# sadPororo/AD-YOLO

Hardware: AMD Instinct MI355X
Metric: train-step audio-sec/s (4ch, se-resnet34+adyolo) (higher is better)
Workload: dtype f32; 1 GPU; se-resnet34 + adyolo loss, synthetic 4ch 24kHz 60s clips, bs=64 per GPU, 12 classes, features+fwd+loss+bwd+allreduce+Adam; global_batch=64, parallelism=dp1

## Files before the change

ad-yolo_amd/_lib.py:

```python
import ctypes
import os

_HERE = os.path.dirname(os.path.abspath(__file__))
LIB_PATH = os.environ.get("ADYOLO_LIB") or os.path.join(_HERE, "libadyolo_hip.so")

P = ctypes.c_void_p
I = ctypes.c_int
L = ctypes.c_long
F = ctypes.c_float
U64 = ctypes.c_uint64

SIGNATURES = {
    "adyolo_abi_version": (I, []),
    "adyolo_last_error": (ctypes.c_char_p, []),
    "adyolo_feat_stft_mel": (I, [P] * 8 + [I, I] + [P] * 4 + [I, I, I, P]),
    "adyolo_feat_finish": (I, [P] * 4 + [I, I, I, P]),
    "adyolo_feat_gcc_phat": (I, [P] * 6 + [I, I, I, I, P]),
    "adyolo_nchw_to_nhwc8": (I, [P, P, I, I, I, I, P]),
    "adyolo_pack_w3x3": (I, [P, P, P, I, I, I, P]),
    "adyolo_conv3x3_tiles": (I, [I] * 3),
    "adyolo_conv3x3_fwd": (I, [P] * 13 + [I] * 7 + [P]),
    "adyolo_wino_pack_w": (I, [P, P, P, I, I, I, P]),
    "adyolo_wino_pack_many": (I, [P, I, I, I, P]),
    "adyolo_wino_tiles": (I, [I] * 3),
    "adyolo_wino_fwd": (I, [P] * 13 + [I] * 7 + [P]),
    "adyolo_wino4_pack_w": (I, [P, P, P, I, I, I, P]),
    "adyolo_wino4_pack_many": (I, [P, I, I, I, P]),
    "adyolo_wino4_tiles": (I, [I] * 3),
    "adyolo_wino4_fwd": (I, [P] * 13 + [I] * 7 + [P]),
    "adyolo_wino4_fwd_form": (I, [I] * 3),
    "adyolo_wino4_last_form": (I, []),
    "adyolo_set_switches": (I, [I]),
    "adyolo_wino4_wgrad_slabs": (I, [I] * 5),
    "adyolo_wino4_wgrad": (I, [P] * 7 + [I] * 6 + [P]),
    "adyolo_wino_wgrad_slabs": (I, [I] * 5),
    "adyolo_wino_wgrad": (I, [P] * 7 + [I] * 6 + [P]),
    "adyolo_conv3x3_wgrad_slabs": (I, [I] * 5),
    "adyolo_conv3x3_wgrad": (I, [P] * 6 + [I] * 6 + [P]),
    "adyolo_wgrad_plan": (I, [I] * 6 + [P]),
    "adyolo_conv_fwd_plan": (I, [I] * 9 + [P]),
    "adyolo_gemm": (I, [P] * 5 + [I] * 10 + [P]),
    "adyolo_gemm_plan": (I, [I] * 8 + [P, P, P]),
    "adyolo_gemm_batched": (I, [P] * 3 + [I] * 10 + [L] * 6 + [F, I, P]),
    "adyolo_colsum": (I, [P, P, P, I, I, I, I, P]),
    "adyolo_bn_stats": (I, [P] * 7 + [I, I, I, F, F, P]),
    "adyolo_bn_stats_tiles": (I, [P] * 11 + [I, I, I, I, F, F, P]),
    "adyolo_bn_eval_stats": (I, [P] * 4 + [I, F, P]),
    "adyolo_bn_scale_shift": (I, [P] * 6 + [I, P]),
    "adyolo_affine_nhwc": (I, [P] * 4 + [L, I, P]),
    "adyolo_bn_bwd_reduce": (I, [P] * 7 + [L, I, P]),
    "adyolo_bn_bwd_tiles": (I, [P, P, P, P, I, I, P]),
    "adyolo_bn_bwd_apply": (I, [P] * 12 + [L, I, I, F, P]),
    "adyolo_bn_persample": (I, [P, P, P, I, I, I, P]),
    "adyolo_bn_finish": (I, [P] * 10 + [I, I, I, F, F, P]),
    "adyolo_se_fc_fwd": (I, [P] * 10 + [I, I, I, I, P]),
    "adyolo_relu_mask_words": (L, [I, I, I]),
    "adyolo_se_tail_fwd": (I, [P] * 9 + [I, I, I, P]),
    "adyolo_se_tail_fwd_pool_ok": (I, [I, I, I]),
    "adyolo_se_tail_fwd_pool": (I, [P] * 9 + [I, I, I, I, P]),
    "adyolo_se_tail_bwd_reduce": (I, [P] * 9 + [I, I, I, P]),
    "adyolo_se_tail_bwd_tiles": (I, [P, P, P, I, I, I, P]),
    "adyolo_se_fc_bwd_words": (L, [I, I]),
    "adyolo_se_fc_bwd": (I, [P] * 16 + [I, I, I, I, P]),
    "adyolo_se_tail_bwd_apply": (I, [P] * 13 + [I, I, I, F, P]),
    "adyolo_se_tail_bwd_reduce_pooled": (I, [P] * 8 + [I, I, I, I, P]),
    "adyolo_se_tail_bwd_apply_pooled": (I, [P] * 13 + [I, I, I, I, F, P]),
    "adyolo_avgpool2_fwd": (I, [P, P, I, I, I, I, P]),
    "adyolo_avgpool2_bwd": (I, [P, P, I, I, I, I, P]),
    "adyolo_add": (I, [P, P, P, L, P]),
    "adyolo_mul": (I, [P, P, P, L, P]),
    "adyolo_scale_dev": (I, [P, P, P, L, P]),
# ... 145 lines not shown
```

ad-yolo_amd/csrc/conv.hip:

```cpp
#include <stdlib.h>
#include "common.hpp"

namespace adyolo {

template <int KC, int BN, int TW>
struct ConvCfg {
    static constexpr int TH = 256 / TW;
    static constexpr int HW_ = TW + 2;
    static constexpr int HH_ = TH + 2;
    static constexpr int NPIX = HW_ * HH_;
    static constexpr int AS = KC + 4;
    static constexpr int NT = BN / 32;
    static constexpr int Q = KC / 4;
    static constexpr int A_FLOATS = NPIX * AS;
    static constexpr int W_FLOATS = BN * AS;
    static constexpr int WPT = (BN * Q + 255) / 256;
};

template <int KC, int BN, int TW>
__global__ __launch_bounds__(256, 2) void conv3x3_fwd_kernel(
    const float *__restrict__ x, const float *__restrict__ wpk, const float *__restrict__ bias,
    const float *__restrict__ addend, const float *__restrict__ addend_mask, const float *__restrict__ in_scale,
    const float *__restrict__ in_shift, float *__restrict__ y, float *__restrict__ stats,
    const float *__restrict__ stat_aux, const float *__restrict__ stat_mean, const float *__restrict__ stat_invstd,
// ... 372 lines not shown
                    float sq = v * v;
                    asm volatile("" : "+v"(sq));
                    ssq += sq;
                }
            }
            float *yrow = y + (((size_t)n * H + gy) * W + tx0) * 32;
#pragma unroll
            for (int k = 0; k < 4; ++k) {
                const int px = k * 8 + (lane >> 3), c4 = lane & 7;
                const f32x4 v4 = *reinterpret_cast<const f32x4 *>(&ot[px * 36 + c4 * 4]);
                if (tx0 + px < W) __builtin_nontemporal_store(v4, reinterpret_cast<f32x4 *>(yrow + (size_t)px * 32 + c4 * 4));
            }
        }
    }
    if (stats) {
        const float a0 = ssum + __shfl_xor(ssum, 32, 64), a1 = ssq + __shfl_xor(ssq, 32, 64);
        if (lh == 0) {
            red[(wave * 32 + li) * 2 + 0] = a0;
            red[(wave * 32 + li) * 2 + 1] = a1;
        }
        __syncthreads();
        if (tid < 64) {
            const int c = tid >> 1, which = tid & 1;
            const float v = red[(0 * 32 + c) * 2 + which] + red[(1 * 32 + c) * 2 + which] + red[(2 * 32 + c) * 2 + which] +
                            red[(3 * 32 + c) * 2 + which];
            stats[which * ((size_t)gridDim.x * 32) + (size_t)blockIdx.x * 32 + c] = v;
        }
    }
}

constexpr int SW_U = 8;
constexpr int SW_T = 64;
constexpr int SW_XS = (SW_T + 4) * 8;
__global__ __launch_bounds__(256, 2) void stem_wgrad_kernel(const float *__restrict__ x, const float *__restrict__ dy,
                                                            float *__restrict__ slabs, int H, int W, int rows_total) {
    __shared__ __attribute__((aligned(16))) float lds[4 * SW_T * 32 + 7 * SW_XS];
    static_assert(4 * SW_T * 32 + 7 * SW_XS >= 4 * 32 * 72, "the reduction buffer must fit");
    float *dyL = lds, *xL = lds + 4 * SW_T * 32;
    const int tid = threadIdx.x, lane = tid & 63, wave = tid >> 6;
    const int li = lane & 31, lh = lane >> 5;
    int ky[3], boff[3];
#pragma unroll
    for (int t = 0; t < 3; ++t) {
        const int n = t * 32 + li, tap = n < 72 ? n >> 3 : 8;
        ky[t] = tap / 3 - 1;
        boff[t] = (lh + 1 + (tap % 3 - 1)) * 8 + (n & 7);
    }
    f32x16 acc[3];
#pragma unroll
    for (int t = 0; t < 3; ++t)
#pragma unroll
        for (int r = 0; r < 16; ++r) acc[t][r] = 0.f;
    for (int i = tid; i < SW_XS; i += 256) xL[6 * SW_XS + i] = 0.f;

    const int per = (rows_total + gridDim.x - 1) / gridDim.x;
    const int r0 = blockIdx.x * per, r1 = min(rows_total, r0 + per);
    const int ncol = (W + SW_T - 1) / SW_T;
    const int nchunk = r0 < r1 ? ((r1 - r0 + 3) / 4) * ncol : 0;
    f32x4 pd[8], px_[4];
    auto request = [&](int chunk) {
        const int cr = r0 + (chunk / ncol) * 4, c0 = (chunk % ncol) * SW_T;
        const __amdgpu_buffer_rsrc_t drs = __builtin_amdgcn_make_buffer_rsrc(const_cast<float *>(dy) + (size_t)cr * W * 32, 0,
                                                                              0x7fffffff, 0x00020000);
        const __amdgpu_buffer_rsrc_t xrs = __builtin_amdgcn_make_buffer_rsrc(const_cast<float *>(x) + ((ptrdiff_t)cr - 1) * W * 8, 0,
                                                                              0x7fffffff, 0x00020000);
#pragma unroll
        for (int i = 0; i < 8; ++i) {
            const int f = tid + 256 * i;
            const int j = f >> 9, col = c0 + ((f & 511) >> 3);
            const bool ok = cr + j < r1 && col < W;
            pd[i] = __builtin_bit_cast(f32x4, __builtin_amdgcn_raw_buffer_load_b128(
                                                  drs, ok ? ((j * W + col) * 32 + (f & 7) * 4) * 4 : (int)0x80000000, 0, 0));
        }
#pragma unroll
        for (int i = 0; i < 4; ++i) {
            const int f = tid + 256 * i;
            const int j = f / 132, rem = f - j * 132;
            const int row = cr - 1 + j, col = c0 - 1 + (rem >> 1);
            const bool ok = f < 6 * 132 && row >= 0 && row < rows_total && col >= 0 && col < W;
            px_[i] = __builtin_bit_cast(f32x4, __builtin_amdgcn_raw_buffer_load_b128(
                                                   xrs, ok ? ((j * W + col) * 8 + (rem & 1) * 4) * 4 : (int)0x80000000, 0, 0));
        }
    };
    auto deposit = [&]() {
#pragma unroll
        for (int i = 0; i < 8; ++i) *reinterpret_cast<f32x4 *>(&dyL[(tid + 256 * i) * 4]) = pd[i];
#pragma unroll
        for (int i = 0; i < 4; ++i) {
            const int f = tid + 256 * i;
            const int j = f / 132;
            if (f < 6 * 132) *reinterpret_cast<f32x4 *>(&xL[j * SW_XS + (f - j * 132) * 4]) = px_[i];
        }
    };
    if (nchunk > 0) request(0);
    for (int chunk = 0; chunk < nchunk; ++chunk) {
        deposit();
        __syncthreads();
        if (chunk + 1 < nchunk) request(chunk + 1);
        const int row = r0 + (chunk / ncol) * 4 + wave;
        if (row < r1) {
            const int y = row % H;
            const float *ap = dyL + (wave * SW_T + lh) * 32 + li;
            const float *bp[3];
#pragma unroll
            for (int t = 0; t < 3; ++t) {
                const int yy = y + ky[t];
                bp[t] = xL + ((yy >= 0 && yy < H) ? wave + 1 + ky[t] : 6) * SW_XS + boff[t];
            }
            constexpr int NG = SW_T / (2 * SW_U);
            float a[2][SW_U], b[2][3][SW_U];
            auto reads = [&](int g) {
#pragma unroll
                for (int u = 0; u < SW_U; ++u) {
                    a[g & 1][u] = ap[(g * SW_U + u) * 64];
#pragma unroll
                    for (int t = 0; t < 3; ++t) b[g & 1][t][u] = bp[t][(g * SW_U + u) * 16];
                }
            };
            reads(0);
#pragma unroll
            for (int g = 0; g < NG; ++g) {
                __builtin_amdgcn_sched_barrier(0);
                if (g + 1 < NG) reads(g + 1);
                __builtin_amdgcn_sched_barrier(0);
#pragma unroll
                for (int u = 0; u < SW_U; ++u)
#pragma unroll
                    for (int t = 0; t < 3; ++t) acc[t] = mfma32(a[g & 1][u], b[g & 1][t][u], acc[t]);
            }
        }
        __syncthreads();
    }
    float *red = lds;
#pragma unroll
    for (int t = 0; t < 3; ++t)
#pragma unroll
        for (int r = 0; r < 16; ++r) {
            const int n = t * 32 + li;
            if (n < 72) red[(wave * 32 + mfma_row(r, lane)) * 72 + n] = acc[t][r];
        }
    __syncthreads();
    for (int i = tid; i < 32 * 72; i += 256)
        slabs[(size_t)blockIdx.x * (32 * 72) + i] = ((red[i] + red[32 * 72 + i]) + red[2 * 32 * 72 + i]) + red[3 * 32 * 72 + i];
}

__global__ __launch_bounds__(256) void conv3x3_wgrad_reduce_kernel(const float *__restrict__ slabs,
                                                                   float *__restrict__ dw, int nslab, int Cout,
                                                                   int CinP, int Cin_real) {
    __shared__ double red[256];
    const int total = Cout * 9 * CinP;
    const double sum = block_colsum32(slabs, nslab, (size_t)total, blockIdx.x * 32, total, red);
    const int idx = blockIdx.x * 32 + (threadIdx.x & 31);
    if ((threadIdx.x >> 5) != 0 || idx >= total) return;
    const int ci = idx % CinP;
    const int tap = (idx / CinP) % 9;
    const int co = idx / (CinP * 9);
    if (ci < Cin_real) dw[((size_t)co * Cin_real + ci) * 9 + tap] = (float)sum;
}

__global__ void pack_w3x3_kernel(const float *__restrict__ w, float *__restrict__ wf,
                                 float *__restrict__ wd, int Cout, int Cin_real, int Cin) {
    const int idx = blockIdx.x * blockDim.x + threadIdx.x;
    if (idx >= Cout * 9 * Cin) return;
    const int ci = idx % Cin;
    const int tap = (idx / Cin) % 9;
    const int co = idx / (Cin * 9);
    const float v = ci < Cin_real ? w[((size_t)co * Cin_real + ci) * 9 + tap] : 0.f;
    wf[idx] = v;
    if (wd) wd[((size_t)ci * 9 + (8 - tap)) * Cout + co] = v;
}

template <int KC, int BN, int TW>
static int launch_fwd(const float *x, const float *wpk, const float *bias, const float *addend,
                      const float *addend_mask, const float *in_scale, const float *in_shift, float *y, float *stats,
                      const float *stat_aux, const float *stat_mean, const float *stat_invstd, const float *stat_mask,
                      int N, int H, int W, int Cin, int Cout, int relu, int mask_bits, hipStream_t st, int tilesW, int tilesH) {
    dim3 grid((unsigned)(N * tilesH * tilesW), (unsigned)(Cout / BN));
    hipLaunchKernelGGL((conv3x3_fwd_kernel<KC, BN, TW>), grid, dim3(256), 0, st, x, wpk, bias, addend, addend_mask,
                       in_scale, in_shift, y, stats, stat_aux, stat_mean, stat_invstd, stat_mask, H, W, Cin, Cout, tilesW,
                       tilesH, relu, mask_bits);
    return check_launch("conv3x3_fwd");
}

static int wgrad_splits(int N, int H, int W, int Cin, int Cout, int *TWo) {
    const int TW = W >= 32 ? 32 : 16, TH = 256 / TW;
    const int ntiles = N * cdiv(H, TH) * cdiv(W, TW);
    const int blocks = (Cout / 32) * cdiv(Cin, 32);
    int nsplit = 1024 / blocks;
    if (nsplit < 1) nsplit = 1;
// ... 56 lines not shown
    hipStream_t st = as_stream(stream);
    const ConvFwdVariant v = conv3x3_fwd_variant(H, W, Cin, Cout, !addend && !in_scale && !stat_aux && !stat_mask);
#define ADYOLO_FWD(KC_, BN_, TW_) \
    launch_fwd<KC_, BN_, TW_>(x, wpk, bias, addend, addend_mask, in_scale, in_shift, y, stats, stat_aux, stat_mean, \
                              stat_invstd, stat_mask, N, H, W, Cin, Cout, relu, mask_bits, st, v.tilesW, v.tilesH)
    if (v.stem) {
        hipLaunchKernelGGL(stem_fwd_kernel, dim3((unsigned)(N * v.tilesH * v.tilesW)), dim3(256), 0, st, x, wpk, bias, y, stats, H,
                           W, v.tilesW, v.tilesH, relu);
        return check_launch("stem_fwd");
    }
    const bool wide = v.TW == 32;
    if (v.KC == 8) return wide ? ADYOLO_FWD(8, 32, 32) : ADYOLO_FWD(8, 32, 16);
    if (v.BN == 64) return wide ? ADYOLO_FWD(32, 64, 32) : ADYOLO_FWD(32, 64, 16);
    return wide ? ADYOLO_FWD(32, 32, 32) : ADYOLO_FWD(32, 32, 16);
#undef ADYOLO_FWD
}

extern "C" int adyolo_conv3x3_wgrad_slabs(int N, int H, int W, int Cin, int Cout) {
    if (N <= 0 || H <= 0 || W <= 0 || Cin <= 0 || Cout <= 0 || Cout % 32) return ADYOLO_EINVAL;
    return wgrad_splits(N, H, W, Cin, Cout, nullptr);
}

extern "C" int adyolo_conv3x3_wgrad(const float *x, const float *dy, const float *in_scale, const float *in_shift,
                                    float *slabs, float *dw, int N, int H, int W, int Cin, int Cin_real, int Cout,
                                    void *stream) {
    ADYOLO_REQUIRE(x && dy && slabs && dw && N > 0 && H > 0 && W > 0, ADYOLO_EINVAL, "conv3x3_wgrad: bad arguments");
    ADYOLO_REQUIRE((Cin == 8 || Cin % 32 == 0) && Cout % 32 == 0 && Cin_real <= Cin, ADYOLO_ENOSUP,
                   "conv3x3_wgrad: unsupported channels Cin=%d Cout=%d", Cin, Cout);
    hipStream_t st = as_stream(stream);
    int TW;
    const int nsplit = wgrad_splits(N, H, W, Cin, Cout, &TW);
    if (Cin == 8 && Cout == 32 && !in_scale && (long)N * H < (1L << 31)) {
        const int nblk = nsplit < 512 ? nsplit : 512;
        hipLaunchKernelGGL(stem_wgrad_kernel, dim3(nblk), dim3(256), 0, st, x, dy, slabs, H, W, N * H);
        int rcs = check_launch("stem_wgrad");
        if (rcs) return rcs;
        hipLaunchKernelGGL(conv3x3_wgrad_reduce_kernel, dim3(cdiv(32 * 72, 32)), dim3(256), 0, st, slabs, dw, nblk, 32, 8,
                           Cin_real);
        return check_launch("stem_wgrad_reduce");
    }
    const int TH = 256 / TW;
    const int tilesW = cdiv(W, TW), tilesH = cdiv(H, TH);
    const int ntiles = N * tilesW * tilesH;
    const int cinBlocks = cdiv(Cin, 32);
    dim3 grid((unsigned)nsplit, (unsigned)((Cout / 32) * cinBlocks));
    if (TW == 32)
        hipLaunchKernelGGL((conv3x3_wgrad_kernel<32>), grid, dim3(256), 0, st, x, dy, in_scale, in_shift, slabs, H, W,
                           Cin, Cout, tilesW, tilesH, ntiles, nsplit, cinBlocks);
    else
        hipLaunchKernelGGL((conv3x3_wgrad_kernel<16>), grid, dim3(256), 0, st, x, dy, in_scale, in_shift, slabs, H, W,
                           Cin, Cout, tilesW, tilesH, ntiles, nsplit, cinBlocks);
    int rc = check_launch("conv3x3_wgrad");
    if (rc) return rc;
    const int CinP = cinBlocks * 32;
    const int total = Cout * 9 * CinP;
    hipLaunchKernelGGL(conv3x3_wgrad_reduce_kernel, dim3(cdiv(total, 32)), dim3(256), 0, st, slabs, dw, nsplit,
                       Cout, CinP, Cin_real);
    return check_launch("conv3x3_wgrad_reduce");
}

extern "C" int adyolo_wgrad_plan(int form, int N, int H, int W, int Cin, int Cout, int *out8) {
    ADYOLO_REQUIRE(out8 && form >= 0 && form <= 3 && N > 0 && H > 0 && W > 0 && Cin > 0 && Cout > 0, ADYOLO_EINVAL,
                   "wgrad_plan: bad arguments");
    for (int i = 0; i < 8; ++i) out8[i] = 0;
    if (form <= 1) {
        if (Cout % 32 || (Cin != 8 && Cin % 32)) return 0;
        if (form == 1 && !(Cin == 8 && Cout == 32 && (long)N * H < (1L << 31))) return 0;
        int TW;
        const int nsplit = wgrad_splits(N, H, W, Cin, Cout, &TW);
        out8[0] = nsplit;
        out8[2] = 1;
        out8[4] = 1;
        if (form == 0) {
            out8[1] = N * cdiv(H, 256 / TW) * cdiv(W, TW);
            out8[3] = 256 / TW;
            out8[5] = TW;
        } else {
            const int nblk = nsplit < 512 ? nsplit : 512;
            out8[1] = N * H;
            out8[3] = cdiv(N * H, nblk);
            out8[5] = SW_T;
            out8[6] = nblk;
        }
        out8[7] = 1;
        return 0;
    }
    if (form == 2) {
        if (adyolo_wino_wgrad_slabs(N, H, W, Cin, Cout) <= 0 ||
            (size_t)H * W * (Cin > Cout ? Cin : Cout) * 4 >= ((size_t)1 << 31))
            return 0;
        wino_wgrad_plan(N, H, W, Cin, Cout, out8);
// ... 73 lines not shown
```

ad-yolo_amd/functional.py:

```python
import os
from typing import NamedTuple

import torch

from . import ops

FUSE_BNBWD = os.environ.get("ADYOLO_FUSE_BNBWD", "1") != "0"
FUSE_POOL = os.environ.get("ADYOLO_FUSE_POOL", "1") != "0"
FUSE_POOL_BWD = os.environ.get("ADYOLO_FUSE_POOL_BWD", "1") != "0"


class BlockLink:

    def __init__(self):
        self.cc = self.mean2 = self.invstd2 = self.tiles = self.ebits = None
        self.affine = self.stem_bn = None
        self.prepooled = None


class BlockArgs(NamedTuple):
    bn1: object
    bn2: object
    bnd: object = None
    link_in: object = None
# ... 157 lines not shown
        if training:
            a, st = ops.conv3x3(x8, wpk, w.shape[0], bias=b, relu=True, want_stats=True)
            _, mean, invstd, scale, shift = _BNState(bn).stats_tiles(st, a, affine=(gamma, beta))
        else:
            a = ops.conv3x3(x8, wpk, w.shape[0], bias=b, relu=True)
            mean, invstd, scale, shift = _BNState(bn).eval_affine(gamma, beta)
        ctx.holder = None
        if holder is not None:
            holder.affine = (scale, shift)
            if training and FUSE_BNBWD:
                holder.stem_bn = (a.detach(), mean, invstd)
                ctx.holder = holder
            out = a
        else:
            out = ops.affine(a, scale, shift)
        ctx.training = training
        ctx.cin_real = w.shape[1]
        ctx.ptrs = (w.data_ptr(), gamma.data_ptr(), beta.data_ptr())
        ctx.wshape = tuple(w.shape)
        ctx.saved_names = ["x8", "a", "gamma", "mean", "invstd"]
        ctx.save_for_backward(x8, a, gamma, mean, invstd)
        return out

    @staticmethod
    def backward(ctx, dout):
        if not ctx.training:
            raise NotImplementedError("backward through eval-mode BatchNorm is not part of the hot path")
        x8, a, gamma, mean, invstd = ctx.saved_tensors
        pw, pg, pb = ctx.ptrs
        vg, vb, vw = SINK.view(pg), SINK.view(pb), SINK.view(pw, ctx.wshape)
        tiles = None
        if ctx.holder is not None and ctx.holder.tiles is not None:
            tiles, ctx.holder.tiles = ctx.holder.tiles, None
        da, dgamma, dbeta, db = ops.bn_bwd(_c(dout), a, gamma, mean, invstd, relu_mask=True, tile_stats=tiles,
                                           out_dgamma=vg, out_dbeta=vb, want_dx_colsum=True)
        dw = ops.conv3x3_wgrad(x8, da, ctx.cin_real, out=vw)
        if vw is not None:
            SINK.done(pw, pg, pb)
            return None, None, db, None, None, None, None, None
        return None, dw, db, dgamma, dbeta, None, None, None


class SEBlockFn(torch.autograd.Function):

    @staticmethod
    def forward(ctx, x, training, pool, args, w1, g1, b1, w2, g2, b2, fw1, fb1, fw2, fb2, wd=None, gd=None, bd=None):
        link_in, link_out, p_aff = args.link_in, args.link_out, args.in_affine
        prepooled = pool and link_in is not None and link_in.prepooled is not None
        if prepooled and tuple(x.shape[1:3]) != link_in.prepooled:
            raise ValueError("SEBlockFn: link_in.prepooled says the block below wrote a %d x %d map, but the input is %d x %d"
                             % (link_in.prepooled + tuple(x.shape[1:3])))
        if p_aff is not None and (pool or wd is not None):
            raise NotImplementedError("p_affine is only supported for identity-shortcut blocks without pooling")
        p = ops.avgpool2(x) if (pool and not prepooled) else x
        n, h, w_, cin = p.shape
        c = w1.shape[0]
        if args.packs is not None:
            wpk1, wpk1d, wpk2, wpk2d = args.packs
        else:
            wpk1, wpk1d = ops.pack_w3x3(w1, cin)
            wpk2, wpk2d = ops.pack_w3x3(w2, c)
        if training:
            a, st1 = ops.conv3x3(p, wpk1, c, relu=True, want_stats=True, in_affine=p_aff)
            _, mean1, invstd1, scale1, shift1 = _BNState(args.bn1).stats_tiles(st1, a, affine=(g1, b1))
        else:
            a = ops.conv3x3(p, wpk1, c, relu=True, in_affine=p_aff)
            mean1, invstd1, scale1, shift1 = _BNState(args.bn1).eval_affine(g1, b1)
        cc, st2 = ops.conv3x3(a, wpk2, c, in_affine=(scale1, shift1), want_stats=True)
        if training:
# ... 646 lines not shown
```

ad-yolo_amd/ops.py:

```python
import ctypes
import os

import numpy as np
import torch

from . import _lib

_c = _lib.call
NULL = ctypes.c_void_p(0)


def _p(t):
    if t is None:
        return NULL
    return ctypes.c_void_p(t.data_ptr())


def _stream():
    return ctypes.c_void_p(torch.cuda.current_stream().cuda_stream)


def _chk(*ts):
    for t in ts:
        if t is None:
# ... 84 lines not shown
    if ts:
        torch.cuda.current_stream(ts[0].device).synchronize()
    return outs


PARAMS_EPOCH = [0]


def params_changed():
    PARAMS_EPOCH[0] += 1


def conv_algo():
    a = os.environ.get("ADYOLO_CONV_ALGO", "winograd4").lower()
    if a not in ("winograd4", "winograd", "direct"):
        raise _lib.AdyoloHipError("ADYOLO_CONV_ALGO must be 'winograd4', 'winograd' or 'direct' (got %r)" % a)
    return a


W4_THRESHOLDS = {}
_THRESHOLD_KEYS = ("min_k", "min_k_addend", "min_wgs", "min_wgrad_work", "min_k_32")


def reload_thresholds():
    env = os.environ.get
    W4_THRESHOLDS.update(min_k=int(env("ADYOLO_W4_MIN_K", "32")),
                         min_k_addend=int(env("ADYOLO_W4_MIN_K_ADDEND", "32")),
                         min_wgs=int(env("ADYOLO_W4_MIN_WGS", "200")),
                         min_wgrad_work=int(env("ADYOLO_W4W_MIN_WORK", "6000000")),
                         min_k_32=int(env("ADYOLO_W4_MIN_K_32", "32")),
                         persist=env("ADYOLO_W4_PERSIST", "1") != "0",
                         narrow=env("ADYOLO_W4_NARROW", "1") != "0",
                         wino1d=env("ADYOLO_WINO1D", "1") != "0",
                         wgrad_algo=(env("ADYOLO_WGRAD_ALGO") or "").lower() or None)
    if _lib.loaded():
        _push_switches(_lib.load())
    return {k: W4_THRESHOLDS[k] for k in _THRESHOLD_KEYS}


def _push_switches(lib):
    lib.adyolo_set_switches((1 if W4_THRESHOLDS["persist"] else 0) | (2 if W4_THRESHOLDS["narrow"] else 0))


_lib.ON_LOAD.append(_push_switches)


def switch_table():
    t = dict(W4_THRESHOLDS)
    t["conv_algo"] = conv_algo()
    return t


def switch_stamp():
    return tuple(sorted((k, str(v)) for k, v in switch_table().items()))


reload_thresholds()

DISPATCH_LOG = None


def w4_narrow_ok(cin, cout):
    return (conv_algo() == "winograd4" and cin % 64 == 0 and cout % 64 == 0 and _w4_eligible(cin, cout) and _w4_eligible(cout, cin)
            and W4_THRESHOLDS["narrow"] and W4_THRESHOLDS["persist"])


def _w4_eligible(k_gemm, n_gemm, allow32=False):
# ... 324 lines not shown
    c = x.shape[-1]
    y = torch.empty_like(x)
    _c("adyolo_affine_nhwc", _p(x), _p(scale), _p(shift), _p(y), x.numel() // c, c, _stream())
    return y


def bn_bwd(dy, x, gamma, mean, invstd, relu_mask=False, tile_stats=None, out_dgamma=None, out_dbeta=None,
           want_dx_colsum=False):
    _chk(dy, x, gamma, mean, invstd)
    c = x.shape[-1]
    rows = x.numel() // c
    sdy = out_dbeta if out_dbeta is not None else _new(x, c)
    sdyx = out_dgamma if out_dgamma is not None else _new(x, c)
    if tile_stats is not None:
        _c("adyolo_bn_bwd_tiles", _p(tile_stats), _p(sdy), _p(sdyx), _p(_new(tile_stats, 2, 256, c)), tile_stats.shape[1], c,
           _stream())
    else:
        partial = _new(x, 2 * 1024 * c)
        _c("adyolo_bn_bwd_reduce", _p(dy), _p(x), _p(mean), _p(invstd), _p(sdy), _p(sdyx), _p(partial), rows, c,
           _stream())
    dx = torch.empty_like(x)
    colsum = part = None
    if want_dx_colsum:
        colsum, part = _new(x, c), _new(x, 8192, c)
    a_sdy, a_sdyx, cs = sdy, sdyx, 1.0
    if EXACT.on:
        glob = EXACT.all_reduce(torch.stack([sdy, sdyx]))
        a_sdy, a_sdyx, cs = glob[0], glob[1], float(EXACT.world)
    _c("adyolo_bn_bwd_apply", _p(dy), _p(x), _p(gamma), _p(mean), _p(invstd), _p(a_sdy), _p(a_sdyx), _p(dx), NULL, NULL,
       _p(colsum), _p(part), rows, c, int(relu_mask), cs, _stream())
    if want_dx_colsum:
        return dx, sdyx, sdy, colsum
    return dx, sdyx, sdy


def se_fc_fwd(ssum, scale, shift, w1, b1, w2, b2, hw):
    _chk(ssum, scale, shift, w1, b1, w2, b2)
    n, c = ssum.shape
    cr = w1.shape[0]
    pooled, hid, s = _new(ssum, n, c), _new(ssum, n, cr), _new(ssum, n, c)
    _c("adyolo_se_fc_fwd", _p(ssum), _p(scale), _p(shift), _p(w1), _p(b1), _p(w2), _p(b2), _p(pooled), _p(hid), _p(s),
       n, hw, c, cr, _stream())
    return pooled, hid, s


def se_tail_pool_ok(h, w, ch):
    return bool(_lib.load().adyolo_se_tail_fwd_pool_ok(int(h), int(w), int(ch)))


def se_tail_fwd(c_t, r_t, scale, shift, s, want_mask=False, r_affine=None, pool_hw=None):
    _chk(c_t, r_t, scale, shift, s)
    n, ch = c_t.shape[0], c_t.shape[-1]
    hw = c_t.numel() // (n * ch)
    mask = None
    if want_mask:
        words = _lib.load().adyolo_relu_mask_words(n, hw, ch)
        if words > 0:
            mask = torch.empty(words, dtype=torch.int64, device=c_t.device)
    rs, rt = r_affine if r_affine is not None else (None, None)
    if pool_hw is not None:
        h, w = pool_hw
        if want_mask and mask is None:
            raise _lib.AdyoloHipError("se_tail_fwd(pool_hw=): the shape has no mask bits")
        pooled = _new(c_t, n, h // 2, w // 2, ch)
        _c("adyolo_se_tail_fwd_pool", _p(c_t), _p(r_t), _p(scale), _p(shift), _p(s), _p(rs), _p(rt), _p(pooled), _p(mask), n, h, w,
           ch, _stream())
# ... 1452 lines not shown
```

include/adyolo_hip.h:

```cpp
#ifndef ADYOLO_HIP_H
#define ADYOLO_HIP_H

#include <stddef.h>
#include <stdint.h>

#ifdef __cplusplus
extern "C" {
#endif

#define ADYOLO_ABI_VERSION 4
#define ADYOLO_EINVAL (-1)
#define ADYOLO_ENOSUP (-2)

int         adyolo_abi_version(void);
const char *adyolo_last_error(void);

int adyolo_feat_stft_mel(const float *audio, const int64_t *clip_offset, const float *twiddle,
                         const int32_t *chunk_mel, const int32_t *chunk_start, const int32_t *chunk_len,
                         const int32_t *chunk_off, const float *mel_w, int n_chunks, int n_mel_w,
                         const float *scaler_mean, const float *scaler_rstd, float *out, float *chan_max, int B,
                         int n_samples, int layout, void *stream);
int adyolo_feat_finish(float *out, const float *chan_max, const float *scaler_mean,
                       const float *scaler_rstd, int B, int T, int layout, void *stream);

// ... 16 lines not shown
int adyolo_wino_tiles(int N, int H, int W);
int adyolo_wino_fwd(const float *x, const float *u, const float *bias, const float *addend,
                    const float *addend_mask, const float *in_scale, const float *in_shift, float *y, float *stats,
                    const float *stat_aux, const float *stat_mean, const float *stat_invstd, const float *stat_mask,
                    int N, int H, int W, int Cin, int Cout, int relu, int mask_bits, void *stream);
int adyolo_wino4_pack_w(const float *w , float *u_fwd , float *u_dgrad ,
                        int Cout, int Cin_real, int Cin, void *stream);
int adyolo_wino4_pack_many(const int64_t *table, int n, int max_cout, int max_cin, void *stream);
int adyolo_wino4_tiles(int N, int H, int W);
int adyolo_wino4_fwd(const float *x, const float *u, const float *bias, const float *addend, const float *addend_mask,
                     const float *in_scale, const float *in_shift, float *y, float *stats, const float *stat_aux,
                     const float *stat_mean, const float *stat_invstd, const float *stat_mask, int N, int H, int W, int Cin,
                     int Cout, int relu, int mask_bits, void *stream);
#define ADYOLO_W4_STATS 1
#define ADYOLO_W4_ADDEND 2
#define ADYOLO_W4_ADDEND_MASK 4
#define ADYOLO_W4_STAT_AUX 8
#define ADYOLO_W4_STAT_MASK 16
#define ADYOLO_W4_BIAS 32
int adyolo_wino4_fwd_form(int Cout, int operands, int mask_bits);
int adyolo_wino4_last_form(void);
int adyolo_set_switches(int bits);
int adyolo_wino4_wgrad_slabs(int N, int H, int W, int Cin, int Cout);
int adyolo_wino4_wgrad(const float *x, const float *dy, const float *in_scale , const float *in_shift ,
                       float *slabs, float *du , float *dw, int N, int H, int W, int Cin, int Cin_real,
                       int Cout, void *stream);
int adyolo_wino_wgrad_slabs(int N, int H, int W, int Cin, int Cout);
int adyolo_wino_wgrad(const float *x, const float *dy, const float *in_scale, const float *in_shift, float *slabs,
                      float *du, float *dw, int N, int H, int W, int Cin, int Cin_real, int Cout, void *stream);
int adyolo_conv3x3_wgrad_slabs(int N, int H, int W, int Cin, int Cout);
int adyolo_conv3x3_wgrad(const float *x, const float *dy, const float *in_scale, const float *in_shift,
                         float *slabs, float *dw, int N, int H, int W, int Cin, int Cin_real, int Cout,
                         void *stream);
int adyolo_wgrad_plan(int form, int N, int H, int W, int Cin, int Cout, int *out8);
int adyolo_conv_fwd_plan(int form, int N, int H, int W, int Cin, int Cout, int operands, int mask_bits, int affine, int *out24);

int adyolo_gemm(const float *A, const float *B, const float *bias, float *C, float *slabs, int M,
                int N, int K, int lda, int ldb, int ldc, int transA, int transB, int splits,
                int accumulate, void *stream);
int adyolo_gemm_plan(int M, int N, int K, int lda, int ldb, int transA, int transB, int splits, int *klen,
                     int *eff_splits, int *fastg);
int adyolo_gemm_batched(const float *A, const float *B, float *C, int M, int N, int K, int lda, int ldb, int ldc,
                        int transA, int transB, int outer, int inner, long oA, long iA, long oB, long iB, long oC,
                        long iC, float alpha, int accumulate, void *stream);
int adyolo_colsum(const float *A, float *out, float *partial, int R, int C, int lda, int accumulate,
                  void *stream);

int adyolo_bn_stats(const float *x, float *ssum, float *mean, float *invstd, float *running_mean,
                    float *running_var, float *partial, int N, int HW, int C, float momentum,
                    float eps, void *stream);
int adyolo_bn_stats_tiles(const float *tile_stats, float *ssum, float *mean, float *invstd, float *running_mean,
                          float *running_var, const float *gamma, const float *beta, float *scale, float *shift,
                          float *partial, int N, int G, int HW, int C, float momentum, float eps, void *stream);
int adyolo_bn_persample(const float *tile_stats, float *ps0, float *ps1, int N, int G, int C, void *stream);
int adyolo_bn_finish(const float *ps0, const float *ps1, float *mean, float *invstd, float *running_mean,
                     float *running_var, const float *gamma, const float *beta, float *scale, float *shift, int N,
                     int HW, int C, float momentum, float eps, void *stream);
int adyolo_bn_eval_stats(const float *running_mean, const float *running_var, float *mean,
                         float *invstd, int C, float eps, void *stream);
int adyolo_bn_scale_shift(const float *gamma, const float *beta, const float *mean,
                          const float *invstd, float *scale, float *shift, int C, void *stream);
int adyolo_affine_nhwc(const float *x, const float *scale, const float *shift, float *y, long rows,
                       int C, void *stream);
int adyolo_bn_bwd_reduce(const float *dy, const float *x, const float *mean, const float *invstd,
                         float *sdy, float *sdyx, float *partial, long rows, int C, void *stream);
int adyolo_bn_bwd_tiles(const float *tile_stats, float *sdy, float *sdyx, float *partial , int tiles, int C,
// ... 319 lines not shown
```

Before: 36400 audio-s/s.

## Fuse stem BN/ReLU backward apply into the stem weight-gradient kernel

The stem's batch-norm backward apply (ReLU mask, normalisation correction) now runs inside the stem wgrad kernel while it loads dy, and the kernel also accumulates the bias gradient. A dedicated reduce kernel sums the wgrad slabs and the bias-gradient partials. This avoids writing and re-reading the full-resolution da tensor and drops a separate apply launch, which matters at the highest-resolution layer. The cost is an extra load stream for the pre-activation in the wgrad kernel, more LDS, and a halved MFMA group unroll that may reduce overlap.

```diff
diff --git a/ad-yolo_amd/_lib.py b/ad-yolo_amd/_lib.py
--- a/ad-yolo_amd/_lib.py
+++ b/ad-yolo_amd/_lib.py
@@ -37,6 +37,8 @@
     "adyolo_wino_wgrad": (I, [P] * 7 + [I] * 6 + [P]),
     "adyolo_conv3x3_wgrad_slabs": (I, [I] * 5),
     "adyolo_conv3x3_wgrad": (I, [P] * 6 + [I] * 6 + [P]),
+    "adyolo_stem_wgrad_bn_ok": (I, [I] * 5),
+    "adyolo_stem_wgrad_bn": (I, [P] * 12 + [I] * 6 + [F, P]),
     "adyolo_wgrad_plan": (I, [I] * 6 + [P]),
     "adyolo_conv_fwd_plan": (I, [I] * 9 + [P]),
     "adyolo_gemm": (I, [P] * 5 + [I] * 10 + [P]),
diff --git a/ad-yolo_amd/csrc/conv.hip b/ad-yolo_amd/csrc/conv.hip
--- a/ad-yolo_amd/csrc/conv.hip
+++ b/ad-yolo_amd/csrc/conv.hip
@@ -428,11 +428,19 @@
 constexpr int SW_U = 8;
 constexpr int SW_T = 64;
 constexpr int SW_XS = (SW_T + 4) * 8;
+struct StemBnArgs {
+    const float *a, *gamma, *mean, *invstd, *sdy, *sdyx;
+    float *dbpart;
+    float invR;
+};
+template <bool BN>
 __global__ __launch_bounds__(256, 2) void stem_wgrad_kernel(const float *__restrict__ x, const float *__restrict__ dy,
-                                                            float *__restrict__ slabs, int H, int W, int rows_total) {
-    __shared__ __attribute__((aligned(16))) float lds[4 * SW_T * 32 + 7 * SW_XS];
+                                                            float *__restrict__ slabs, int H, int W, int rows_total,
+                                                            const StemBnArgs bn) {
+    __shared__ __attribute__((aligned(16))) float lds[4 * SW_T * 32 + 7 * SW_XS + (BN ? 5 * 32 + 256 * 4 : 0)];
     static_assert(4 * SW_T * 32 + 7 * SW_XS >= 4 * 32 * 72, "the reduction buffer must fit");
     float *dyL = lds, *xL = lds + 4 * SW_T * 32;
+    const float *parL = lds + 4 * SW_T * 32 + 7 * SW_XS;
     const int tid = threadIdx.x, lane = tid & 63, wave = tid >> 6;
     const int li = lane & 31, lh = lane >> 5;
     int ky[3], boff[3];
@@ -454,19 +462,37 @@
     const int ncol = (W + SW_T - 1) / SW_T;
     const int nchunk = r0 < r1 ? ((r1 - r0 + 3) / 4) * ncol : 0;
     f32x4 pd[8], px_[4];
+    f32x4 pa[BN ? 8 : 1];
+    f32x4 *dbL = reinterpret_cast<f32x4 *>(lds + 4 * SW_T * 32 + 7 * SW_XS + 5 * 32) + tid;
+    unsigned okbits = 0;
+    if constexpr (BN) {
+        if (tid < 5 * 32) {
+            const float *src[5] = {bn.gamma, bn.mean, bn.invstd, bn.sdy, bn.sdyx};
+            lds[4 * SW_T * 32 + 7 * SW_XS + tid] = src[tid >> 5][tid & 31];
+        }
+        *dbL = f32x4{0.f, 0.f, 0.f, 0.f};
+        __syncthreads();
+    }
     auto request = [&](int chunk) {
         const int cr = r0 + (chunk / ncol) * 4, c0 = (chunk % ncol) * SW_T;
         const __amdgpu_buffer_rsrc_t drs = __builtin_amdgcn_make_buffer_rsrc(const_cast<float *>(dy) + (size_t)cr * W * 32, 0,
                                                                               0x7fffffff, 0x00020000);
         const __amdgpu_buffer_rsrc_t xrs = __builtin_amdgcn_make_buffer_rsrc(const_cast<float *>(x) + ((ptrdiff_t)cr - 1) * W * 8, 0,
                                                                               0x7fffffff, 0x00020000);
+        if constexpr (BN) okbits = 0;
 #pragma unroll
         for (int i = 0; i < 8; ++i) {
             const int f = tid + 256 * i;
             const int j = f >> 9, col = c0 + ((f & 511) >> 3);
             const bool ok = cr + j < r1 && col < W;
-            pd[i] = __builtin_bit_cast(f32x4, __builtin_amdgcn_raw_buffer_load_b128(
-                                                  drs, ok ? ((j * W + col) * 32 + (f & 7) * 4) * 4 : (int)0x80000000, 0, 0));
+            const int off = ok ? ((j * W + col) * 32 + (f & 7) * 4) * 4 : (int)0x80000000;
+            pd[i] = __builtin_bit_cast(f32x4, __builtin_amdgcn_raw_buffer_load_b128(drs, off, 0, 0));
+            if constexpr (BN) {
+                const __amdgpu_buffer_rsrc_t ars = __builtin_amdgcn_make_buffer_rsrc(
+                    const_cast<float *>(bn.a) + (size_t)cr * W * 32, 0, 0x7fffffff, 0x00020000);
+                pa[i] = __builtin_bit_cast(f32x4, __builtin_amdgcn_raw_buffer_load_b128(ars, off, 0, 0));
+                okbits |= (ok ? 1u : 0u) << i;
+            }
         }
 #pragma unroll
         for (int i = 0; i < 4; ++i) {
@@ -479,8 +505,29 @@
         }
     };
     auto deposit = [&]() {
-#pragma unroll
-        for (int i = 0; i < 8; ++i) *reinterpret_cast<f32x4 *>(&dyL[(tid + 256 * i) * 4]) = pd[i];
+        f32x4 dbacc;
+        if constexpr (BN) dbacc = *dbL;
+#pragma unroll
+        for (int i = 0; i < 8; ++i) {
+            if constexpr (BN) {
+                const int cq = (tid & 7) * 4;
+                const f32x4 gis = *reinterpret_cast<const f32x4 *>(parL + cq), mq = *reinterpret_cast<const f32x4 *>(parL + 32 + cq);
+                const f32x4 isq = *reinterpret_cast<const f32x4 *>(parL + 64 + cq), sa = *reinterpret_cast<const f32x4 *>(parL + 96 + cq);
+                const f32x4 sb = *reinterpret_cast<const f32x4 *>(parL + 128 + cq);
+                const f32x4 d = pd[i], xv = pa[i];
+                const bool ok = (okbits >> i) & 1u;
+                f32x4 o;
+#pragma unroll
+                for (int k = 0; k < 4; ++k) {
+                    o[k] = gis[k] * isq[k] * (d[k] - sa[k] * bn.invR - (xv[k] - mq[k]) * isq[k] * sb[k] * bn.invR);
+                    if (!(ok && xv[k] > 0.f)) o[k] = 0.f;
+                    dbacc[k] += o[k];
+                }
+                pd[i] = o;
+            }
+            *reinterpret_cast<f32x4 *>(&dyL[(tid + 256 * i) * 4]) = pd[i];
+        }
+        if constexpr (BN) *dbL = dbacc;
 #pragma unroll
         for (int i = 0; i < 4; ++i) {
             const int f = tid + 256 * i;
@@ -503,14 +550,15 @@
                 const int yy = y + ky[t];
                 bp[t] = xL + ((yy >= 0 && yy < H) ? wave + 1 + ky[t] : 6) * SW_XS + boff[t];
             }
-            constexpr int NG = SW_T / (2 * SW_U);
-            float a[2][SW_U], b[2][3][SW_U];
+            constexpr int GU = BN ? SW_U / 2 : SW_U;
+            constexpr int NG = SW_T / (2 * GU);
+            float a[2][GU], b[2][3][GU];
             auto reads = [&](int g) {
 #pragma unroll
-                for (int u = 0; u < SW_U; ++u) {
-                    a[g & 1][u] = ap[(g * SW_U + u) * 64];
-#pragma unroll
-                    for (int t = 0; t < 3; ++t) b[g & 1][t][u] = bp[t][(g * SW_U + u) * 16];
+                for (int u = 0; u < GU; ++u) {
+                    a[g & 1][u] = ap[(g * GU + u) * 64];
+#pragma unroll
+                    for (int t = 0; t < 3; ++t) b[g & 1][t][u] = bp[t][(g * GU + u) * 16];
                 }
             };
             reads(0);
@@ -520,7 +568,7 @@
                 if (g + 1 < NG) reads(g + 1);
                 __builtin_amdgcn_sched_barrier(0);
 #pragma unroll
-                for (int u = 0; u < SW_U; ++u)
+                for (int u = 0; u < GU; ++u)
 #pragma unroll
                     for (int t = 0; t < 3; ++t) acc[t] = mfma32(a[g & 1][u], b[g & 1][t][u], acc[t]);
             }
@@ -536,6 +584,13 @@
             if (n < 72) red[(wave * 32 + mfma_row(r, lane)) * 72 + n] = acc[t][r];
         }
     __syncthreads();
+    if constexpr (BN) {
+        if (tid < 8) {
+            f32x4 t = dbL[0];
+            for (int k = 8; k < 256; k += 8) t += dbL[k];
+            *reinterpret_cast<f32x4 *>(bn.dbpart + (size_t)blockIdx.x * 32 + tid * 4) = t;
+        }
+    }
     for (int i = tid; i < 32 * 72; i += 256)
         slabs[(size_t)blockIdx.x * (32 * 72) + i] = ((red[i] + red[32 * 72 + i]) + red[2 * 32 * 72 + i]) + red[3 * 32 * 72 + i];
 }
@@ -551,6 +606,24 @@
     const int ci = idx % CinP;
     const int tap = (idx / CinP) % 9;
     const int co = idx / (CinP * 9);
+    if (ci < Cin_real) dw[((size_t)co * Cin_real + ci) * 9 + tap] = (float)sum;
+}
+
+__global__ __launch_bounds__(256) void stem_wgrad_bn_reduce_kernel(const float *__restrict__ slabs, const float *__restrict__ dbpart,
+                                                                   float *__restrict__ dw, float *__restrict__ db, int nslab,
+                                                                   int Cin_real) {
+    __shared__ double red[256];
+    constexpr int total = 32 * 72;
+    const int cx = threadIdx.x & 31;
+    if (blockIdx.x == total / 32) {
+        const double sum = block_colsum32(dbpart, nslab, 32, 0, 32, red);
+        if ((threadIdx.x >> 5) == 0) db[cx] = (float)sum;
+        return;
+    }
+    const double sum = block_colsum32(slabs, nslab, (size_t)total, blockIdx.x * 32, total, red);
+    const int idx = blockIdx.x * 32 + cx;
+    if ((threadIdx.x >> 5) != 0) return;
+    const int ci = idx % 8, tap = (idx / 8) % 9, co = idx / 72;
     if (ci < Cin_real) dw[((size_t)co * Cin_real + ci) * 9 + tap] = (float)sum;
 }
 
@@ -673,7 +746,7 @@
     const int nsplit = wgrad_splits(N, H, W, Cin, Cout, &TW);
     if (Cin == 8 && Cout == 32 && !in_scale && (long)N * H < (1L << 31)) {
         const int nblk = nsplit < 512 ? nsplit : 512;
-        hipLaunchKernelGGL(stem_wgrad_kernel, dim3(nblk), dim3(256), 0, st, x, dy, slabs, H, W, N * H);
+        hipLaunchKernelGGL((stem_wgrad_kernel<false>), dim3(nblk), dim3(256), 0, st, x, dy, slabs, H, W, N * H, StemBnArgs{});
         int rcs = check_launch("stem_wgrad");
         if (rcs) return rcs;
         hipLaunchKernelGGL(conv3x3_wgrad_reduce_kernel, dim3(cdiv(32 * 72, 32)), dim3(256), 0, st, slabs, dw, nblk, 32, 8,
@@ -698,6 +771,32 @@
     hipLaunchKernelGGL(conv3x3_wgrad_reduce_kernel, dim3(cdiv(total, 32)), dim3(256), 0, st, slabs, dw, nsplit,
                        Cout, CinP, Cin_real);
     return check_launch("conv3x3_wgrad_reduce");
+}
+
+extern "C" int adyolo_stem_wgrad_bn_ok(int N, int H, int W, int Cin, int Cout) {
+    return N > 0 && H > 0 && W > 0 && Cin == 8 && Cout == 32 && (long)N * H < (1L << 31) && (long)W * 4 * 32 * 4 < (1L << 31);
+}
+
+extern "C" int adyolo_stem_wgrad_bn(const float *x, const float *dout, const float *a, const float *gamma, const float *mean,
+                                    const float *invstd, const float *sdy, const float *sdyx, float *slabs, float *dbpart,
+                                    float *dw, float *db, int N, int H, int W, int Cin, int Cin_real, int Cout,
+                                    float count_scale, void *stream) {
+    ADYOLO_REQUIRE(x && dout && a && gamma && mean && invstd && sdy && sdyx && slabs && dbpart && dw && db && Cin_real > 0 &&
+                       Cin_real <= Cin && count_scale >= 1.f,
+                   ADYOLO_EINVAL, "stem_wgrad_bn: bad arguments");
+    ADYOLO_REQUIRE(adyolo_stem_wgrad_bn_ok(N, H, W, Cin, Cout), ADYOLO_ENOSUP,
+                   "stem_wgrad_bn: only the 8 -> 32 channel stem (N=%d H=%d W=%d Cin=%d Cout=%d)", N, H, W, Cin, Cout);
+    ADYOLO_REQUIRE(((uintptr_t)x | (uintptr_t)dout | (uintptr_t)a | (uintptr_t)dbpart) % 16 == 0, ADYOLO_EINVAL,
+                   "stem_wgrad_bn: x, dout, a and dbpart must be 16-byte aligned");
+    hipStream_t st = as_stream(stream);
+    const int nsplit = wgrad_splits(N, H, W, Cin, Cout, nullptr);
+    const int nblk = nsplit < 512 ? nsplit : 512;
+    StemBnArgs bn = {a, gamma, mean, invstd, sdy, sdyx, dbpart, (float)(1.0 / ((double)N * H * W * (double)count_scale))};
+    hipLaunchKernelGGL((stem_wgrad_kernel<true>), dim3(nblk), dim3(256), 0, st, x, dout, slabs, H, W, N * H, bn);
+    int rc = check_launch("stem_wgrad_bn");
+    if (rc) return rc;
+    hipLaunchKernelGGL(stem_wgrad_bn_reduce_kernel, dim3(32 * 72 / 32 + 1), dim3(256), 0, st, slabs, dbpart, dw, db, nblk, Cin_real);
+    return check_launch("stem_wgrad_bn_reduce");
 }
 
 extern "C" int adyolo_wgrad_plan(int form, int N, int H, int W, int Cin, int Cout, int *out8) {
diff --git a/ad-yolo_amd/functional.py b/ad-yolo_amd/functional.py
--- a/ad-yolo_amd/functional.py
+++ b/ad-yolo_amd/functional.py
@@ -213,9 +213,13 @@
         tiles = None
         if ctx.holder is not None and ctx.holder.tiles is not None:
             tiles, ctx.holder.tiles = ctx.holder.tiles, None
-        da, dgamma, dbeta, db = ops.bn_bwd(_c(dout), a, gamma, mean, invstd, relu_mask=True, tile_stats=tiles,
-                                           out_dgamma=vg, out_dbeta=vb, want_dx_colsum=True)
-        dw = ops.conv3x3_wgrad(x8, da, ctx.cin_real, out=vw)
+        if ops.stem_bwd_fused_ok(x8, a):
+            dw, dgamma, dbeta, db = ops.stem_bwd_fused(x8, _c(dout), a, gamma, mean, invstd, ctx.cin_real, tile_stats=tiles,
+                                                       out_dw=vw, out_dgamma=vg, out_dbeta=vb)
+        else:
+            da, dgamma, dbeta, db = ops.bn_bwd(_c(dout), a, gamma, mean, invstd, relu_mask=True, tile_stats=tiles,
+                                               out_dgamma=vg, out_dbeta=vb, want_dx_colsum=True)
+            dw = ops.conv3x3_wgrad(x8, da, ctx.cin_real, out=vw)
         if vw is not None:
             SINK.done(pw, pg, pb)
             return None, None, db, None, None, None, None, None
diff --git a/ad-yolo_amd/ops.py b/ad-yolo_amd/ops.py
--- a/ad-yolo_amd/ops.py
+++ b/ad-yolo_amd/ops.py
@@ -140,7 +140,8 @@
                          persist=env("ADYOLO_W4_PERSIST", "1") != "0",
                          narrow=env("ADYOLO_W4_NARROW", "1") != "0",
                          wino1d=env("ADYOLO_WINO1D", "1") != "0",
-                         wgrad_algo=(env("ADYOLO_WGRAD_ALGO") or "").lower() or None)
+                         wgrad_algo=(env("ADYOLO_WGRAD_ALGO") or "").lower() or None,
+                         fuse_stem_bnbwd=env("ADYOLO_FUSE_STEM_BNBWD", "1") != "0")
     if _lib.loaded():
         _push_switches(_lib.load())
     return {k: W4_THRESHOLDS[k] for k in _THRESHOLD_KEYS}
@@ -531,6 +532,43 @@
     if want_dx_colsum:
         return dx, sdyx, sdy, colsum
     return dx, sdyx, sdy
+
+
+def stem_bwd_fused_ok(x8, a):
+    n, h, w, cin = x8.shape
+    cout = a.shape[-1]
+    return bool(W4_THRESHOLDS["fuse_stem_bnbwd"] and wgrad_form(cin, cout, None, (n, h, w))[0] == "conv3x3_wgrad_kernel"
+                and _lib.load().adyolo_stem_wgrad_bn_ok(n, h, w, cin, cout))
+
+
+def stem_bwd_fused(x8, dout, a, gamma, mean, invstd, cin_real, tile_stats=None, out_dw=None, out_dgamma=None, out_dbeta=None):
+    _chk(x8, dout, a, gamma, mean, invstd)
+    n, h, w, cin = x8.shape
+    c = a.shape[-1]
+    sdy = out_dbeta if out_dbeta is not None else _new(a, c)
+    sdyx = out_dgamma if out_dgamma is not None else _new(a, c)
+    if tile_stats is not None:
+        _c("adyolo_bn_bwd_tiles", _p(tile_stats), _p(sdy), _p(sdyx), _p(_new(tile_stats, 2, 256, c)), tile_stats.shape[1], c,
+           _stream())
+    else:
+        partial = _new(a, 2 * 1024 * c)
+        _c("adyolo_bn_bwd_reduce", _p(dout), _p(a), _p(mean), _p(invstd), _p(sdy), _p(sdyx), _p(partial), a.numel() // c, c,
+           _stream())
+    a_sdy, a_sdyx, cs = sdy, sdyx, 1.0
+    if EXACT.on:
+        glob = EXACT.all_reduce(torch.stack([sdy, sdyx]))
+        a_sdy, a_sdyx, cs = glob[0], glob[1], float(EXACT.world)
+    nslab = _lib.load().adyolo_conv3x3_wgrad_slabs(n, h, w, cin, c)
+    if nslab <= 0:
+        raise _lib.AdyoloHipError("conv3x3_wgrad_slabs rejected the shape")
+    dw = out_dw if out_dw is not None else _new(a, c, cin_real, 3, 3)
+    db, slabs, dbpart = _new(a, c), _new(a, nslab, c, 9, 32), _new(a, nslab, c)
+    if DISPATCH_LOG is not None:
+        k = ("conv3x3_wgrad_kernel", cin, c, 0)
+        DISPATCH_LOG[k] = DISPATCH_LOG.get(k, 0) + 1
+    _c("adyolo_stem_wgrad_bn", _p(x8), _p(dout), _p(a), _p(gamma), _p(mean), _p(invstd), _p(a_sdy), _p(a_sdyx), _p(slabs),
+       _p(dbpart), _p(dw), _p(db), n, h, w, cin, cin_real, c, cs, _stream())
+    return dw, sdyx, sdy, db
 
 
 def se_fc_fwd(ssum, scale, shift, w1, b1, w2, b2, hw):
diff --git a/include/adyolo_hip.h b/include/adyolo_hip.h
--- a/include/adyolo_hip.h
+++ b/include/adyolo_hip.h
@@ -72,6 +72,10 @@
 int adyolo_conv3x3_wgrad(const float *x, const float *dy, const float *in_scale, const float *in_shift,
                          float *slabs, float *dw, int N, int H, int W, int Cin, int Cin_real, int Cout,
                          void *stream);
+int adyolo_stem_wgrad_bn_ok(int N, int H, int W, int Cin, int Cout);
+int adyolo_stem_wgrad_bn(const float *x, const float *dout, const float *a, const float *gamma, const float *mean,
+                         const float *invstd, const float *sdy, const float *sdyx, float *slabs, float *dbpart, float *dw,
+                         float *db , int N, int H, int W, int Cin, int Cin_real, int Cout, float count_scale, void *stream);
 int adyolo_wgrad_plan(int form, int N, int H, int W, int Cin, int Cout, int *out8);
 int adyolo_conv_fwd_plan(int form, int N, int H, int W, int Cin, int Cout, int operands, int mask_bits, int affine, int *out24);
 
```

After: 36600 audio-s/s (median of 6 runs). Within noise of the previous version (+0.6%).
